# yangye1098/Speech-Denoising-Diffusion-Model-2

Hardware: AMD Instinct MI355X
Metric: denoised audio sec/sec, 1000-step UNetModified2 @16kHz (higher is better)
Workload: dtype bf16; 1 GPU; UNetModified2 config_unet.json, linear 1e-6..1e-3, T=1000, 16x16448-sample chunks per GPU, condition_in; model=UNetModified2, global_batch=16, seq_len=16448, parallelism=dp1, lane_rows=16

## Files before the change

### speech-denoising-diffusion-model-2_amd/csrc/conv_deep.hip

```cpp
#include "conv_common.h"
#include "conv_tile_cfg.h"
#include "kernels.h"

namespace sddm {

__device__ __attribute__((aligned(256))) unsigned char g_deep_zero[256];

constexpr int kDeepMaxChunks = 10;

#ifdef SDDM_STAMPS_ISSUE
#define DS_W(a) SDDM_STAMP(a, 1)
#define DS_STG(a) SDDM_STAMP(a, 2)
#define DS_ISSUED(a) SDDM_STAMP(a, 3)
#define DS_LANDED(a) SDDM_STAMP(a, 4)
#define DS_XFORM(a) SDDM_STAMP(a, 5)
#define DS_KLOOP(a) SDDM_STAMP(a, 6)
#define DS_STORED(a) do {} while (0)
#define DS_STATS(a) do {} while (0)
#else
#define DS_W(a) do {} while (0)
#define DS_STG(a) do {} while (0)
#define DS_ISSUED(a) SDDM_STAMP(a, 1)
#define DS_LANDED(a) SDDM_STAMP(a, 2)
#define DS_XFORM(a) SDDM_STAMP(a, 3)
// ... 62 lines not shown
    {128, 0, 8, 16, 32, 16, 96, 96, 96, 0, 0, 0, 1, 0, 8, 32, 0},
    {128, 0, 8, 16, 32, 16, 96, 0, 96, 96, 96, 2, 1, 0, 4, 32, 0},
    {64, 1, 4, 16, 64, 16, 96, 0, 96, 0, 0, 0, 0, 0, 4, 32, 1},
    {64, 0, 8, 8, 32, 8, 128, 0, 160, 0, 0, 0, 1, 0, 4, 32, 1},
    {64, 0, 8, 8, 32, 8, 160, 0, 160, 128, 0, 2, 1, 0, 4, 32, 1},
    {32, 1, 8, 4, 16, 4, 160, 0, 160, 0, 0, 0, 0, 0, 4, 32, 1},
    {32, 0, 8, 4, 16, 4, 160, 0, 160, 0, 0, 0, 1, 0, 4, 32, 1},
    {32, 0, 8, 4, 16, 4, 160, 0, 160, 0, 0, 1, 1, 0, 4, 32, 1},
    {32, 0, 8, 4, 16, 4, 160, 160, 160, 0, 0, 0, 1, 0, 4, 32, 1},
    {32, 0, 8, 4, 16, 4, 160, 0, 160, 160, 160, 2, 1, 0, 4, 32, 1},
    {64, 0, 8, 8, 32, 8, 160, 0, 160, 0, 0, 0, 0, 1, 4, 32, 1},
};
static constexpr int kNDeepShapes = (int)(sizeof(kDeepShapes) / sizeof(kDeepShapes[0]));

template <typename T, bool S2, int MT, int NW, int D, int NB, int SH>
__global__ __launch_bounds__(64 * NW, 8 / NW) void conv_deep_kernel(ConvArgs a) {
  extern __shared__ __attribute__((aligned(16))) char smem[];
  constexpr ConvShape SC = kDeepShapes[SH];
  constexpr bool CS = SH > 0;
  SDDM_SHAPE_GEO(SC, CS, S2, a)
  constexpr int NT = 64 * NW;
  constexpr int ES = (int)sizeof(T);
  constexpr int UPP = 2 * ES;
  constexpr int UPL = ES / 2;
  constexpr int VE = 16 / ES;
  constexpr int FP = MT / 16, FC = NB / 16, NBP = NB + 4;
  constexpr int TPP = NB / 4;
  constexpr int PPI = NT / TPP;
  constexpr int EIT = (MT + PPI - 1) / PPI;
  static_assert(NB == 16 || NB == 32 || NB == 64, "16, 32 or 64 output channels per block");
  constexpr int SLOTS = (NW == 8 && MT >= 128) ? 4 : NW;

  int tile, b, zb;
  if (a.deep_zin) xcd_block<true>(gNT, gCout / NB, tile, b, zb);
  else xcd_block<false>(gNT, gCout / NB, tile, b, zb);
  const int tid = threadIdx.x, lane = tid & 63, g = lane >> 4;
  const int wv = __builtin_amdgcn_readfirstlane(tid >> 6);
  const int n0 = zb * NB;
  const int ty = tile / gTX, tx = tile - ty * gTX;
  const int y0 = ty * gTR, x0 = tx * gTW;
  const int npv = gTR * gTW;
  const DeepGeo geo = deep_geo(S2, gTR, gTW, MT);
  const int HC = geo.HC, PLB = geo.PLB, PLR = geo.PLR;
  const int Cin = gCA + gCB, nck = Cin / 32, npl = Cin / VE, plA = gCA / VE;
  const int RC = gRes == 2 ? gRCA + gRCB : 0, rck = RC / 32, nplr = RC / VE, plRA = gRCA / VE;
  const bool gn = gGN, ident = gRes == 1;
  const DeepLds lay = deep_layout<T, MT, NW, NB>(geo, Cin, RC);
  float* gsc = (float*)(smem + lay.gsc);
  const int res_off = npl * PLB;
  const int img_in = gHi * gWi, img_out = gHo * gWo;
  const char* srcA = (const char*)a.srcA + (size_t)b * img_in * gCA * ES;
  const char* srcB = (const char*)(gCB ? a.srcB : a.srcA) + (size_t)b * img_in * gCB * ES;
  const char* zero = (const char*)g_deep_zero;
  const int* tdp = a.t_dev ? a.t_dev : (const int*)g_deep_zero;
  const int t_step = *tdp;
  const int t_now = a.temb_per_b ? b : t_step;
  SDDM_STAMP(a, 0);

  const int ec4 = (tid & (TPP - 1)) * 4;
  GNLoadT<DeepGN<NW>::GK> gl;
  const GNFuse gf{a.gstA, a.gtilesA, a.gntileA, a.gstB, a.gtilesB, a.gntileB, a.gamma, a.beta, a.groups, a.eps};
  gl.issue(gf, b, gCA, gCB, gn, a.bias);
  const int ns3 = nck * 9, ns = ns3 + rck;
  const int nj = wv < ns ? (ns - wv + NW - 1) / NW : 0;
  const int s_last = wv + NW * max(nj - 1, 0);
  const int cb0 = n0 / 16;
  const T* wbase = (const T*)a.wgt_f + (size_t)lane * 8;
  const T* rbase = (const T*)a.res_wgt_f + (size_t)lane * 8;
  auto wfrag = [&](int s, int fc) -> Frag<T> {
    const T* p = s < ns3 ? wbase + ((size_t)(cb0 + fc) * ns3 + s) * 512
                         : rbase + ((size_t)(cb0 + fc) * rck + (s - ns3)) * 512;
    return load_frag<T>((const char*)p);
  };
  Frag<T> wa[D][FC];
#pragma unroll
  for (int d = 0; d < D; ++d)
#pragma unroll
    for (int fc = 0; fc < FC; ++fc) wa[d][fc] = SDDM_DEEP_DBG(32) ? Frag<T>{} : wfrag(min(wv + NW * d, s_last), fc);
  DS_W(a);
  f32x4 idr[EIT];
  {
    const T* rsrc = (const T*)a.res_src + (size_t)b * img_out * gCout + n0 + ec4;
#pragma unroll
    for (int it = 0; it < EIT; ++it) {
      const int p = min(it * PPI + tid / TPP, npv - 1), py = p / gTW, px = p - py * gTW;
      const T* rp = ident ? rsrc + ((y0 + py) * gWo + (x0 + px)) * gCout : (const T*)g_deep_zero;
      idr[it] = load4<T>(rp);
    }
  }
  auto dma = [&](const char* src, char* dst) {
    __builtin_amdgcn_global_load_lds((const __attribute__((address_space(1))) void*)src,
                                     (__attribute__((address_space(3))) void*)dst, 16, 0, 0);
  };
  unsigned inb = 0;
  {
    const float rHC = 1.0f / (float)HC;
    for (int r = 0; r < geo.NCH; ++r) {
      const int hp = r * 64 + lane, hy = fdivi(hp, rHC), hx = hp - hy * HC;
      int iy, ix;
      bool ok;
      if (S2) {
        iy = 2 * y0 - 1 + hy; ix = 2 * x0 - 1 + hx;
        ok = iy >= 0 && iy < gHi && ix >= 0 && ix < gWi;
      } else {
        iy = y0 - 1 + hy; ix = x0 - 1 + hx;
        ok = iy >= 0 && iy < gHo && ix >= 0 && ix < gWo;
        if (gUp) { iy >>= 1; ix >>= 1; }
      }
      ok = ok && hp < geo.HP;
      inb |= ok ? 1u << r : 0u;
      const unsigned pix = ok ? (unsigned)(iy * gWi + ix) : 0u;
      const char* pa = ok ? srcA + pix * (unsigned)(gCA * ES) : zero;
      const char* pb = ok ? srcB + pix * (unsigned)(gCB * ES) - plA * 16 : zero;
      const unsigned step = ok ? 16u : 0u;
      char* dl = smem + r * 1024;
      for (int q = wv; q < npl; q += NW)
        if (!SDDM_DEEP_DBG(4)) dma((q < plA ? pa : pb) + q * step, dl + q * PLB);
    }
  }
  if (rck) {
    const char* rawA = (const char*)a.rawA + (size_t)b * img_out * gRCA * ES;
    const char* rawB = (const char*)(gRCB ? a.rawB : a.rawA) + (size_t)b * img_out * gRCB * ES;
    for (int r = 0; r < geo.NCR; ++r) {
      const int p = r * 64 + lane, py = p / gTW, px = p - py * gTW;
      const int pix = p < npv ? (y0 + py) * gWo + (x0 + px) : -1;
      const unsigned oa = (unsigned)pix * (unsigned)(gRCA * ES), ob = (unsigned)pix * (unsigned)(gRCB * ES);
      for (int q = wv; q < nplr; q += NW) {
        const char* src = q < plRA ? rawA + oa + q * 16 : rawB + ob + (q - plRA) * 16;
        dma(pix >= 0 ? src : zero, smem + res_off + q * PLR + r * 1024);
      }
    }
  }
  DS_STG(a);
  float bb[4], sshift;
  {
    const float* trow = a.temb ? a.temb + (size_t)t_now * a.temb_ld : a.bias;
#pragma unroll
    for (int i = 0; i < 4; ++i) {
      const float bv = a.bias[n0 + ec4 + i], tv = trow[n0 + ec4 + i];
      bb[i] = bv + (a.temb ? tv : 0.f);
    }
    const int cs = n0 + (tid & (NB - 1));
    const float sbv = a.bias[cs], stv = trow[cs];
    sshift = sbv + (a.temb ? stv : 0.f);
  }
  DS_ISSUED(a);

  if (gn) gl.finish(gf, b, gCA, gCB, gsc, gsc + Cin);
  dma_sync();
  DS_LANDED(a);

  if (gn) {
    for (int q0 = wv; q0 < npl; q0 += 2 * NW) {
      const bool two = q0 + NW < npl;
      const int q1 = two ? q0 + NW : q0;
      float s0[VE], h0[VE], s1[VE], h1[VE];
#pragma unroll
      for (int j = 0; j < VE; j += 4) {
        const f32x4 x0 = *(const f32x4*)(gsc + q0 * VE + j), y0 = *(const f32x4*)(gsc + Cin + q0 * VE + j);
        const f32x4 x1 = *(const f32x4*)(gsc + q1 * VE + j), y1 = *(const f32x4*)(gsc + Cin + q1 * VE + j);
#pragma unroll
// ... 58 lines not shown
  }
  DS_KLOOP(a);

  lds_sync();
  float* red = (float*)smem;
  auto put = [&](int slot) {
#pragma unroll
    for (int fp = 0; fp < FP; ++fp) {
      const int p = fp * 16 + (lane & 15);
#pragma unroll
      for (int fc = 0; fc < FC; ++fc) *(f32x4*)(red + (slot * MT + p) * NBP + fc * 16 + 4 * g) = acc[fp][fc];
    }
  };
  if (SLOTS < NW) {
    if (wv >= SLOTS) put(wv - SLOTS);
    lds_sync();
    if (wv < SLOTS) {
#pragma unroll
      for (int fp = 0; fp < FP; ++fp) {
        const int p = fp * 16 + (lane & 15);
#pragma unroll
        for (int fc = 0; fc < FC; ++fc) acc[fp][fc] += *(const f32x4*)(red + (wv * MT + p) * NBP + fc * 16 + 4 * g);
      }
      put(wv);
    }
  } else {
    put(wv);
  }
  lds_sync();

  float sn = 0.f, s1[4], s2[4];
#pragma unroll
  for (int i = 0; i < 4; ++i) { s1[i] = 0.f; s2[i] = 0.f; }
  T* out = (T*)a.out + (size_t)b * img_out * gCout + n0 + ec4;
#pragma unroll
  for (int it = 0; it < EIT; ++it) {
    const int p = it * PPI + tid / TPP;
    if (p < npv) {
      const int py = p / gTW, px = p - py * gTW;
      f32x4 s = *(const f32x4*)(red + p * NBP + ec4);
#pragma unroll
      for (int w = 1; w < SLOTS; ++w) s += *(const f32x4*)(red + (w * MT + p) * NBP + ec4);
      float d[4];
#pragma unroll
      for (int i = 0; i < 4; ++i) d[i] = s[i] + idr[it][i];
      store4<T>(out + ((y0 + py) * gWo + (x0 + px)) * gCout, d[0] + bb[0], d[1] + bb[1], d[2] + bb[2], d[3] + bb[3]);
#pragma unroll
      for (int i = 0; i < 4; ++i) {
        s1[i] += d[i];
        s2[i] += d[i] * d[i];
      }
      sn += 1.f;
    }
  }
  DS_STORED(a);
  if (a.stats) {
    auto wred = [](float x) {
      if constexpr (TPP == 4) x += dpp_f32<0x124>(x);
      if constexpr (TPP <= 8) x += dpp_f32<0x128>(x);
      x += __shfl_xor(x, 16);
      return x + __shfl_xor(x, 32);
    };
    const float tn = wred(sn);
    float t1[4], t2[4];
#pragma unroll
    for (int i = 0; i < 4; ++i) { t1[i] = wred(s1[i]); t2[i] = wred(s2[i]); }
    lds_sync();
    float* xs = red;
    if (lane < TPP)
#pragma unroll
      for (int i = 0; i < 4; ++i) {
        float* e = xs + (wv * NB + ec4 + i) * 3;
        e[0] = tn; e[1] = t1[i]; e[2] = t2[i];
      }
    lds_sync();
    if (tid < NB) {
      float n = 0.f, u1 = 0.f, u2 = 0.f;
#pragma unroll
      for (int r = 0; r < NW; ++r) {
        const float* e = xs + (r * NB + tid) * 3;
        n += e[0]; u1 += e[1]; u2 += e[2];
      }
      float* dst = a.stats + (((size_t)b * gNT + tile) * gCout + n0 + tid) * 2;
      dst[0] = (sshift + u1 / n) * n;
      dst[1] = fmaxf(u2 - u1 * u1 / n, 0.f);
    }
  }
  DS_STATS(a);
  SDDM_STAMP(a, 7);
}

template <typename T, int MT, int NW>
static int deep_ring(int steps_per_wave) {
  if (sizeof(T) == 4 || NW == 4) return 8 / (int)(sizeof(T) == 4 ? 2 : 1);
  if (steps_per_wave <= 8 || MT >= 128) return 8;
  return 12;
}

template <typename T, bool S2, int MT, int NW, int NB, int SH = 0>
static hipError_t deep_go(const ConvArgs& a, int B, hipStream_t s, size_t* lo) {
  const int Cin = a.CA + a.CB, RC = a.res_mode == 2 ? a.RCA + a.RCB : 0;
  const int nck = Cin / 32, rck = RC / 32;
  const DeepGeo geo = deep_geo(S2, a.TR, a.TW, MT);
  const DeepLds lay = deep_layout<T, MT, NW, NB>(geo, Cin, RC);
  const bool fits = geo.NCH <= kDeepMaxChunks && geo.NCR <= 2;
  if (lo) {
    *lo = fits ? (size_t)lay.total : (size_t)1 << 40;
    return hipSuccess;
  }
  if (!fits || a.TR * a.TW > MT || a.Cout % NB || Cin % 32 || Cin > 1000 || RC % 32 || a.CA % 32)
    return hipErrorInvalidValue;
  if (lay.total > kLdsBytes) return hipErrorInvalidValue;
  const dim3 grid = xcd_grid(a.n_tiles, B, a.Cout / NB), blk(64 * NW);
  const int D = deep_ring<T, MT, NW>((nck * 9 + rck + NW - 1) / NW);
#define SDDM_RING(DV)                                                                         \
  if (D == DV) {                                                                              \
    hipLaunchKernelGGL((conv_deep_kernel<T, S2, MT, NW, DV, NB, SH>), grid, blk, lay.total, s, a); \
    return hipGetLastError();                                                                 \
  }
  if constexpr (NB == 64) {
    if constexpr (sizeof(T) == 4) {
      return hipErrorInvalidValue;
    } else {
      hipLaunchKernelGGL((conv_deep_kernel<T, S2, MT, NW, 4, NB, SH>), grid, blk, lay.total, s, a);
      return hipGetLastError();
    }
  } else if constexpr (SH > 0) {
    constexpr ConvShape c = kDeepShapes[SH];
    constexpr int spw = (((c.CA + c.CB) / 32) * 9 + (c.res == 2 ? (c.RCA + c.RCB) / 32 : 0) + NW - 1) / NW;
    constexpr int DS = (NW == 4 || MT >= 128 || spw <= 8) ? 8 : 12;
    SDDM_RING(DS)
  } else if constexpr (sizeof(T) == 4) {
    SDDM_RING(4)
  } else if constexpr (NW == 4 || MT >= 128) {
    SDDM_RING(8)
  } else {
    SDDM_RING(8) SDDM_RING(12)
  }
#undef SDDM_RING
  return hipErrorInvalidValue;
// ... 64 lines not shown
```

### speech-denoising-diffusion-model-2_amd/csrc/kernels.h

```cpp
#pragma once
#include <hip/hip_runtime.h>
#include <stdint.h>

namespace sddm {

struct EmbedArgs {
  const float* noise_levels;
  const float* table;
  int time_step_mode;
  int R;
  int dim;
  const float* emb_vec;
  const float* w1; const float* b1;
  const float* w2; const float* b2;
  const float* pw; const float* pb;
  int SC;
  float* out;
};
hipError_t launch_embed(const EmbedArgs& a, hipStream_t s);

struct GNSrc { const float* stats; int C; int tiles; int n_tile; };
struct GNArgs {
  GNSrc a, b;
  const float* gamma; const float* beta;
// ... 16 lines not shown
};
hipError_t launch_conv_in(int dtype, const ConvInArgs& a, int B, hipStream_t s);

struct GNFuse;
struct ConvArgs {
  const void* srcA; const void* srcB; int CA, CB;
  int Hi, Wi;
  int Ho, Wo;
  int upsample;
  int TR, TW, tiles_x, n_tiles;
  const float* gstA; int gtilesA, gntileA;
  const float* gstB; int gtilesB, gntileB;
  const float* gamma; const float* beta; int groups; float eps;
  const void* wgt;
  const float* bias;
  const float* temb; int temb_ld; const int* t_dev; int temb_per_b;
  int Cout;
  int res_mode;
  const void* res_src;
  const void* rawA; const void* rawB; int RCA, RCB;
  const void* res_wgt;
  void* out;
  float* stats;
  int deep_zin;
  int deep_nw;
  int deep_nb;
  unsigned long long* stamps;
  int dbg;
  const void* wgt_t;
  const void* res_wgt_t;
  const void* wgt_f;
  const void* res_wgt_f;
};

struct ChainArgs {
  const void* x;
  void* out;
  const void* wgt[5];
  const void* res_wgt;
  const float* bias[5];
  const float* gamma[4]; const float* beta[4];
  const float* temb[2];
  int temb_ld; const int* t_dev; int temb_per_b;
  int C, H, W, groups; float eps;
};
hipError_t launch_conv_chain(int dtype, const ChainArgs& a, int B, hipStream_t s);

struct TileCfg { int wpx, wco, fp, fc; };
int conv_tile_ncfg();
TileCfg conv_tile_cfg(int cfg);
hipError_t launch_conv_tile(int dtype, int cfg, bool s2, const ConvArgs& a, int B, hipStream_t s);
size_t conv_tile_lds_bytes(int cfg, bool s2, const ConvArgs& a);

hipError_t launch_conv_deep(int dtype, int mt, bool s2, const ConvArgs& a, int B, hipStream_t s);
size_t conv_deep_lds_bytes(int dtype, int mt, bool s2, const ConvArgs& a);
int conv_deep_ring_depth(int dtype, int mt, int nw, int ksteps, int nb);

constexpr int kLdsBytes = 160 * 1024;

hipError_t launch_conv_strip(int dtype, int nblk, int mpi, int SR, const ConvArgs& a, int B, hipStream_t s);
size_t conv_strip_lds_bytes(int dtype, int nblk, int mpi, const ConvArgs& a);

struct TransCoef {
  const float* betas; const float* alphas; const float* sqrt_alpha_bar; const float* pnc;
  const float* sigma; const float* sgamma; const float* ssh; const float* sqrt_delta;
  const float* c_xt; const float* c_yt; const float* c_epst; const float* sde;
// ... 79 lines not shown
```

### speech-denoising-diffusion-model-2_amd/csrc/sddm_runtime.cpp

```cpp
#include <hip/hip_runtime.h>

#include <algorithm>
#include <cstdarg>
#include <cstdlib>
#include <cstdio>
#include <cstring>
#include <functional>
#include <map>
#include <set>
#include <memory>
#include <string>
#include <vector>

#include "../../include/sddm_hip.h"
#include "json_mini.h"
#include "kernels.h"
#include "q_kernels.h"
#include "stft_kernels.h"
#include "sddm_common.h"

namespace sddm {
int compute_schedule(const std::string& schedule, int T, double linear_start, double linear_end,
                     float* out);
}
// ... 134 lines not shown
      s[n + ".block2.block.0.bias"] = {L.cout};
      s[n + ".block2.block.3.weight"] = {L.cout, L.cout, 3, 3};
      s[n + ".block2.block.3.bias"] = {L.cout};
      if (L.cin != L.cout) {
        s[n + ".res_conv.weight"] = {L.cout, L.cin, 1, 1};
        s[n + ".res_conv.bias"] = {L.cout};
      }
    } else if (L.kind == 2 || L.kind == 3) {
      s[n + ".conv.weight"] = {L.cout, L.cin, 3, 3};
      s[n + ".conv.bias"] = {L.cout};
    } else if (L.kind == 0) {
      s[n + ".weight"] = {L.cout, L.cin, 3, 3};
      s[n + ".bias"] = {L.cout};
    } else {
      s[n + ".block.0.weight"] = {L.cin};
      s[n + ".block.0.bias"] = {L.cin};
      s[n + ".block.3.weight"] = {L.cout, L.cin, 3, 3};
      s[n + ".block.3.bias"] = {L.cout};
    }
  }
  return s;
}

struct Param { std::vector<int64_t> shape; std::vector<float> data; bool loaded = false; };
struct Tensor { void* p = nullptr; int C = 0, H = 0, W = 0; float* stats = nullptr; int tiles = 0, n_tile = 0; };
struct Op {
  int cls;
  double bytes, flops;
  std::function<hipError_t(hipStream_t)> run;
  std::string name = "";
  std::function<hipError_t(hipStream_t, int)> run_dbg = nullptr;
  std::string kname = "";
  std::string kinst = "";
};
struct ProfAcc { double ms = 0; int64_t n = 0; double bytes = 0, flops = 0; };

struct RunState {
  const float* cond = nullptr;
  float* x = nullptr;
  const float* temb = nullptr;
  int temb_per_b = 0;
  int* t_dev = nullptr;
  int final_mode = 0;
  float* eps_out = nullptr;
  uint64_t seed = 0;
  int64_t row_offset = 0;
  const float* noise = nullptr;
  int64_t noise_ld = 0;
};

static constexpr int kStreams = 4;
static constexpr int kMaxLanes = 64;

struct Lane {
  int B = 0, row0 = 0, idx = 0;
  Arena arena;
  std::vector<Op> ops;
  RunState rs;
  size_t off_temb_fwd = 0, off_cond = 0, off_x = 0;
  hipGraphExec_t gexec = nullptr;
  hipGraph_t graph = nullptr;
  int g_K = 0, g_gen = -1;
  ~Lane() {
    if (gexec) (void)hipGraphExecDestroy(gexec);
    if (graph) (void)hipGraphDestroy(graph);
    arena.reset();
// ... 257 lines not shown
    const int TW = std::min(a.Wo, mt);
    if (mt % TW || a.Wo % TW) continue;
    const int TR = std::min(mt / TW, a.Ho);
    if (a.Ho % TR) continue;
    if (TR * TW < mt && mt > 32) continue;
    a.TR = TR; a.TW = TW; a.tiles_x = a.Wo / TW; a.n_tiles = a.tiles_x * (a.Ho / TR);
    for (int nw : {8, 4}) {
      a.deep_nw = nw;
      if (conv_deep_lds_bytes(dt, mt, s2, a) > kLdsBytes) continue;
      const int blocks = a.n_tiles * B * nz, per_round = 256 * (nw == 4 ? 2 : 1);
      cs.push_back({mt, nw, TR, TW, a.tiles_x, a.n_tiles, blocks, (blocks + per_round - 1) / per_round});
    }
  }
  if (cs.empty()) return false;
  const Cand* pick = nullptr;
  const int fm = want_mt ? want_mt : force_mt, fn = want_mt ? want_nw : force_nw;
  for (const Cand& c : cs)
    if (c.mt == fm && c.nw == fn) pick = &c;
  if (!pick) {
    pick = &cs[0];
    for (const Cand& c : cs) {
      if (c.rounds != pick->rounds) { if (c.rounds < pick->rounds) pick = &c; continue; }
      if (c.nw != pick->nw) { if (c.nw > pick->nw) pick = &c; continue; }
      if (c.mt < pick->mt) pick = &c;
    }
  }
  ch.strip = 0; ch.mt = pick->mt; ch.nw = pick->nw; ch.nb = nb; ch.ckb = (a.CA + a.CB) / 32;
  ch.TR = pick->TR; ch.TW = pick->TW; ch.tiles_x = pick->tiles_x; ch.n_tiles = pick->n_tiles;
  return true;
}

static int deep_zin(const ConvArgs& a, int B, size_t es) {
  static const int force = std::getenv("SDDM_DEEP_ZIN") ? std::atoi(std::getenv("SDDM_DEEP_ZIN")) : -1;
  if (force >= 0) return force;
  const double in = (double)B * a.Hi * a.Wi * (a.CA + a.CB) * es;
  const double w = (double)a.Cout * ((a.CA + a.CB) * 9 + (a.res_mode == 2 ? a.RCA + a.RCB : 0)) * es;
  return in >= w ? 1 : 0;
}

static bool choose_tile(int dt, int B, ConvArgs a, bool s2, ConvChoice& ch, int want = -1) {
  if (dt == DT_F32) return false;
  static const int force = std::getenv("SDDM_TILE_CFG") ? std::atoi(std::getenv("SDDM_TILE_CFG")) : -1;
  static const bool off = std::getenv("SDDM_NO_TILE") != nullptr;
  if (off) return false;
  const int fw = want >= 0 ? want : force;
  struct Cand { int cfg, TR, TW, tiles_x, n_tiles, blocks, area; };
  std::vector<Cand> cs;
  for (int cfg = 0; cfg < conv_tile_ncfg(); ++cfg) {
    const TileCfg t = conv_tile_cfg(cfg);
    const int MT = t.wpx * t.fp * 16, NB = t.wco * t.fc * 16;
    if (a.Cout % NB) continue;
    const int TW = std::min(a.Wo, MT);
    if (MT % TW || a.Wo % TW) continue;
    const int TR = std::min(MT / TW, a.Ho);
    if (a.Ho % TR) continue;
    if (TR * TW < MT && (TR != a.Ho || TW != a.Wo)) continue;
    a.TR = TR; a.TW = TW; a.tiles_x = a.Wo / TW; a.n_tiles = a.tiles_x * (a.Ho / TR);
    if (conv_tile_lds_bytes(cfg, s2, a) > kLdsBytes) continue;
    cs.push_back({cfg, TR, TW, a.tiles_x, a.n_tiles, a.n_tiles * B * (a.Cout / NB), TR * TW * NB});
  }
  if (cs.empty()) return false;
  const Cand* pick = nullptr;
  for (const Cand& c : cs)
    if (c.cfg == fw) pick = &c;
  if (!pick) {
    for (const Cand& c : cs) {
      if (!pick) { pick = &c; continue; }
// ... 16 lines not shown
  a.Hi = up ? Ho / 2 : (s2 ? Ho * 2 : Ho); a.Wi = up ? Wo / 2 : (s2 ? Wo * 2 : Wo);
  static const int env_mpi = std::getenv("SDDM_STRIP_MPI") ? std::atoi(std::getenv("SDDM_STRIP_MPI")) : 0;
  static const int env_blocks = std::getenv("SDDM_STRIP_BLOCKS") ? std::atoi(std::getenv("SDDM_STRIP_BLOCKS")) : 0;
  if (kind == 2) {
    ConvChoice t = ch;
    if (choose_tile(dt, B, a, s2, t, ka) && t.tile == ka) { ch = t; return true; }
  }
  if (!s2 && (Wo == 128 || Wo == 64) && std::getenv("SDDM_NO_STRIP") == nullptr && (kind == 0 || kind == 1)) {
    const int nbs[2] = {(Cout % 64 == 0) ? 64 : 32, 32};
    for (int mpi : {256, 128}) {
      if (env_mpi && mpi != env_mpi) continue;
      const int TRs = mpi / Wo;
      if (Ho % TRs) continue;
      for (int ni = 0; ni < 2; ++ni) {
        const int nb = nbs[ni];
        if (conv_strip_lds_bytes(dt, nb, mpi, a) > kLdsBytes) continue;
        const int nz = (Cout + nb - 1) / nb;
        int SR = 0;
        const int target = env_blocks ? env_blocks : 256;
        for (int m = 32; m >= 2; m /= 2) {
          const int sr = TRs * m;
          if (Ho % sr) continue;
          SR = sr;
          if ((Ho / sr) * B * nz >= target) break;
        }
        if (SR == 0) continue;
        ch.strip = 1; ch.nblk = nb; ch.SR = SR; ch.mpi = mpi;
        ch.TR = SR; ch.TW = Wo; ch.tiles_x = 1; ch.n_tiles = Ho / SR;
        return true;
      }
    }
  }
  if (want_mt == 0 && kind != 3 && choose_tile(dt, B, a, s2, ch)) return true;
  return choose_deep(dt, B, a, s2, ch, want_mt, want_nw, want_nb);
}

static int build_lane(sddm_ctx* c, Lane& L) {
  const int B = L.B;
  Lane* lp = &L;
  const int dt = c->dtype;
  const size_t es = dtype_size(dt);
  const UNetCfg& u = c->ucfg;
  const int N = c->num_samples, W = u.seg, S = u.stride;
  const int F = (N - W) / S + 1;
  L.ops.clear();
  L.arena.reset();
  Arena& A = L.arena;

  struct TRes { size_t p, st; int C, H, W, tiles, n_tile; };
  std::vector<TRes> tres;
  auto new_tensor = [&](int C, int H, int Wd, int tiles, int n_tile) -> int {
    TRes t;
    t.p = A.reserve((size_t)B * H * Wd * C * es);
    t.st = A.reserve(sizeof(float) * (size_t)B * tiles * C * 2);
    t.C = C; t.H = H; t.W = Wd; t.tiles = tiles; t.n_tile = n_tile;
    tres.push_back(t);
    return (int)tres.size() - 1;
  };
  struct GNRes { int a, b; std::string w; };
  std::vector<GNRes> gres;
  auto new_gn = [&](int xa, int xb, const std::string& w) -> int {
    gres.push_back({xa, xb, w});
    return (int)gres.size() - 1;
  };
  L.off_temb_fwd = A.reserve(sizeof(float) * (size_t)B * std::max(c->SC, 1));
  L.off_cond = A.reserve(sizeof(float) * (size_t)B * N);
  L.off_x = A.reserve(sizeof(float) * (size_t)B * N);

  enum { ST_CONVIN, ST_GN, ST_CONV, ST_FINAL };
  struct Step {
    int type = 0;
    std::string w;
    std::string rb;
    int srcA = -1, srcB = -1, gn = -1, out = -1;
    int s2 = 0, up = 0, res_mode = 0, rawA = -1, rawB = -1, cout = 0;
    bool temb = false;
    ConvChoice ch;
  };
  std::vector<Step> prog;
  const int PB = std::max(1, c->lane_rows);
  const sddm_ctx::TuneTable* tuned = nullptr;
  for (const auto& tt : c->tunes)
    if (tt.B == PB && tt.N == N && tt.dtype == dt) { tuned = &tt; break; }
  if (!tuned && dt == DT_F16)
    for (const auto& tt : c->tunes)
      if (tt.B == PB && tt.N == N && tt.dtype == DT_BF16) { tuned = &tt; break; }
  auto pick = [&](const std::string& name, int Cin, int RC, int res_mode, int Ho, int Wo, int cout, bool s2, bool up,
                  ConvChoice& ch) {
    int wm = 0, wn = 0, wb = 0, kind = 0, ka = 0;
    if (tuned) {
      auto it = tuned->deep_tune.find(name);
      if (it != tuned->deep_tune.end()) { wm = it->second.first; wn = it->second.second; kind = 3; }
      auto kt = tuned->kern_tune.find(name);
      if (kt != tuned->kern_tune.end()) {
        kind = kt->second.kind; ka = kt->second.a;
        if (kind == 3) { wm = kt->second.a; wn = kt->second.b; wb = kt->second.c; }
      }
    }
    const bool chain = kind == 4 && dt != DT_F32;
    if (kind == 4) kind = 0;
    const bool ok = choose_conv(dt, PB, Cin, RC, res_mode, Ho, Wo, cout, s2, up, ch, wm, wn, kind, ka, wb);
    ch.chain = chain ? 1 : 0;
    return ok;
  };
  const int TRin = 512 / W;
  if (u.inner != 32 || 512 % W || F % TRin || (TRin + 1) * S + W + 2 > 1024)
    FAIL(SDDM_ERR_NOT_IMPLEMENTED, "conv_in needs inner_channel 32 and segment_len dividing 512 (got %d, %d)", u.inner, W);
  const int t0 = new_tensor(u.inner, F, W, F / TRin, TRin * W);
  { Step st; st.type = ST_CONVIN; st.out = t0; prog.push_back(st); }

  auto res_block = [&](const std::string& n, int xa, int xb, int cin, int cout) -> int {
    const int H = tres[xa].H, Wd = tres[xa].W;
    ConvChoice c1, c2;
    if (!pick(n + ".block1", cin, 0, 0, H, Wd, cout, false, false, c1)) return -1;
    if (!pick(n + ".block2", cout, cin, cin != cout ? 2 : 1, H, Wd, cout, false, false, c2)) return -1;
    const int g1 = new_gn(xa, xb, n + ".block1");
    const int h = new_tensor(cout, H, Wd, c1.n_tiles, c1.TR * c1.TW);
    { Step st; st.type = ST_CONV; st.w = n + ".block1"; st.rb = n; st.srcA = xa; st.srcB = xb; st.gn = g1;
      st.out = h; st.cout = cout; st.temb = true; st.ch = c1; prog.push_back(st); }
    const int g2 = new_gn(h, -1, n + ".block2");
    const int o = new_tensor(cout, H, Wd, c2.n_tiles, c2.TR * c2.TW);
    { Step st; st.type = ST_CONV; st.w = n + ".block2"; st.rb = n; st.srcA = h; st.gn = g2; st.out = o;
      st.cout = cout; st.res_mode = cin != cout ? 2 : 1; st.rawA = xa; st.rawB = xb; st.ch = c2; prog.push_back(st); }
    return o;
  };
  std::vector<LayerDesc> downs, mid, ups;
  unet_layers(u, &downs, &mid, &ups);
  std::vector<int> feats{t0};
  int cur = t0;
  for (size_t i = 1; i < downs.size(); ++i) {
    const LayerDesc& L = downs[i];
    if (L.kind == 1) {
// ... 7 lines not shown
      Step st; st.type = ST_CONV; st.w = L.name; st.srcA = cur; st.out = o; st.s2 = 1; st.cout = L.cout; st.ch = ch;
      prog.push_back(st);
      cur = o;
    }
    if (cur < 0) FAIL(SDDM_ERR_SHAPE, "no tile for %s", L.name.c_str());
    feats.push_back(cur);
  }
  for (const LayerDesc& L : mid) {
    cur = res_block(L.name, cur, -1, L.cin, L.cout);
    if (cur < 0) FAIL(SDDM_ERR_SHAPE, "no tile for %s", L.name.c_str());
  }
  for (const LayerDesc& L : ups) {
    if (L.kind == 1) {
      const int skip = feats.back();
      feats.pop_back();
      if (tres[skip].H != tres[cur].H || tres[skip].W != tres[cur].W)
        FAIL(SDDM_ERR_SHAPE, "skip/upsample size mismatch at %s (torch.cat would raise)", L.name.c_str());
      cur = res_block(L.name, cur, skip, L.cin, L.cout);
      if (cur < 0) FAIL(SDDM_ERR_SHAPE, "no tile for %s", L.name.c_str());
    } else {
      const int H = tres[cur].H * 2, Wd = tres[cur].W * 2;
      ConvChoice ch;
      if (!pick(L.name, tres[cur].C, 0, 0, H, Wd, L.cout, false, true, ch)) FAIL(SDDM_ERR_SHAPE, "no tile for %s", L.name.c_str());
      const int o = new_tensor(L.cout, H, Wd, ch.n_tiles, ch.TR * ch.TW);
      Step st; st.type = ST_CONV; st.w = L.name; st.srcA = cur; st.out = o; st.up = 1; st.cout = L.cout; st.ch = ch;
      prog.push_back(st);
      cur = o;
    }
  }
  const int gf = new_gn(cur, -1, "final_conv");
  { Step st; st.type = ST_FINAL; st.srcA = cur; st.gn = gf; prog.push_back(st); }

  SDDM_HIP_CHECK(A.commit());

  auto TT = [&](int i) {
    Tensor t;
    if (i < 0) return t;
    const TRes& r = tres[i];
    t.p = A.base + r.p; t.stats = A.at<float>(r.st); t.C = r.C; t.H = r.H; t.W = r.W;
    t.tiles = r.tiles; t.n_tile = r.n_tile;
    return t;
  };
  auto WF = [&](const std::string& k) { return c->warena.at<float>(c->woff.at(k)); };
  auto WV = [&](const std::string& k) { return (const void*)(c->warena.base + c->woff.at(k)); };
  auto conv_args = [&](const Step& st, ConvArgs& a, double& bytes, double& flops) -> int {
    a = ConvArgs{};
    const Tensor sa = TT(st.srcA), sb = TT(st.srcB), o = TT(st.out);
    a.srcA = sa.p; a.srcB = sb.p; a.CA = sa.C; a.CB = sb.C;
    a.Hi = sa.H; a.Wi = sa.W; a.Ho = o.H; a.Wo = o.W; a.upsample = st.up;
    a.Cout = st.cout; a.out = o.p; a.stats = o.stats;
    if (st.gn >= 0) {
      const GNRes& gr = gres[st.gn];
      const Tensor ga = TT(gr.a), gb = TT(gr.b);
      a.gstA = ga.stats; a.gtilesA = ga.tiles; a.gntileA = ga.n_tile;
      a.gstB = gb.stats; a.gtilesB = gb.tiles; a.gntileB = gb.n_tile;
      a.gamma = WF(gr.w + ".gamma"); a.beta = WF(gr.w + ".beta"); a.groups = u.groups; a.eps = 1e-5f;
      const int Ct = ga.C + gb.C;
      if (Ct % u.groups || (gb.C && ga.C % (Ct / u.groups)) || 256 % u.groups)
        FAIL(SDDM_ERR_SHAPE, "GroupNorm(%d, %d) at %s: unsupported grouping", u.groups, Ct, gr.w.c_str());
    }
    a.wgt = WV(st.w + ".w"); a.bias = WF(st.w + ".b");
    a.wgt_t = c->woff.count(st.w + ".w_t") ? WV(st.w + ".w_t") : nullptr;
    a.wgt_f = WV(st.w + ".w_f");
    a.res_mode = st.res_mode;
    const int Cin = a.CA + a.CB;
    bytes = (double)B * a.Hi * a.Wi * Cin * es + (double)B * a.Ho * a.Wo * a.Cout * es +
// ... 74 lines not shown
      const Tensor o = TT(st.out);
      a.out = o.p; a.stats = o.stats; a.TR = TRin;
      const double bytes = (double)B * N * 4 * 2 + (double)B * F * W * u.inner * es;
      const double flops = 2.0 * B * F * W * u.inner * 18;
#ifdef SDDM_STAMPS
      if (const char* sn = std::getenv("SDDM_STAMPS"))
        if (std::string(sn) == "downs.0") {
          if (!c->stamp_buf) SDDM_HIP_CHECK(hipMalloc(&c->stamp_buf, sizeof(unsigned long long) * 8 * 65536));
          a.stamps = c->stamp_buf;
          c->stamp_blocks = (int64_t)(F / TRin) * B;
        }
#endif
      L.ops.push_back({0, bytes, flops, [lp, a, dt, B](hipStream_t s) {
                          ConvInArgs x = a;
                          x.cond = lp->rs.cond; x.x = lp->rs.x; x.t_dev = lp->rs.t_dev;
                          return launch_conv_in(dt, x, B, s);
                        }, "downs.0"});
      L.ops.back().kname = std::string("conv_in_kernel<") + dt_name(dt) + ">";
      L.ops.back().kinst = L.ops.back().kname;
    } else if (st.type == ST_CONV) {
      ConvArgs a;
      double bytes = 0, flops = 0;
      if (const int r = conv_args(st, a, bytes, flops)) return r;
      const int Cin = a.CA + a.CB;
      const ConvChoice ch = st.ch;
      const bool s2 = st.s2 != 0;
      const bool temb = st.temb;
      if (std::getenv("SDDM_PRINT_SHAPES"))
        fprintf(stderr, "SHAPE %s %s%d s2=%d TR=%d TW=%d Ho=%d Wo=%d CA=%d CB=%d Cout=%d RCA=%d RCB=%d res=%d gn=%d up=%d mt=%d nw=%d nb=%d nblk=%d mpi=%d SR=%d ntiles=%d\n",
                st.w.c_str(), ch.strip ? "strip" : (ch.tile >= 0 ? "tile" : "deep"), ch.tile >= 0 ? ch.tile : ch.mt, s2 ? 1 : 0,
                a.TR, a.TW, a.Ho, a.Wo, a.CA, a.CB, a.Cout, a.RCA, a.RCB, a.res_mode, a.gamma ? 1 : 0, a.upsample ? 1 : 0,
                ch.mt, ch.nw, ch.nb, ch.nblk, ch.mpi, ch.SR, a.n_tiles);
      const int toff = temb ? c->temb_off.at(st.rb) : 0;
#ifdef SDDM_STAMPS
      if (const char* sn = std::getenv("SDDM_STAMPS")) {
        if (st.w == sn) {
          if (!c->stamp_buf) SDDM_HIP_CHECK(hipMalloc(&c->stamp_buf, sizeof(unsigned long long) * 8 * 65536));
          SDDM_HIP_CHECK(hipMemset(c->stamp_buf, 0, sizeof(unsigned long long) * 8 * 65536));
          a.stamps = c->stamp_buf;
          if (const char* f = std::getenv("SDDM_STAMPS_DBG")) a.dbg = std::atoi(f);
          int nb = 32;
          if (ch.tile >= 0) { const TileCfg tc = conv_tile_cfg(ch.tile); nb = tc.wco * tc.fc * 16; }
          c->stamp_blocks = ch.strip ? (int64_t)(a.Ho / ch.SR) * B * ((a.Cout + ch.nblk - 1) / ch.nblk)
                                     : (int64_t)a.n_tiles * B * (a.Cout / (ch.tile >= 0 ? nb : ch.nb));
        }
      }
#endif
      L.ops.push_back({2, bytes, flops, [ctx, lp, a, s2, ch, dt, B, temb, toff](hipStream_t s) {
                          ConvArgs x = a;
                          if (temb) {
                            x.temb = lp->rs.temb + toff;
                            x.temb_ld = ctx->SC;
                            x.temb_per_b = lp->rs.temb_per_b;
                            x.t_dev = lp->rs.t_dev;
                          }
                          if (ch.strip) return launch_conv_strip(dt, ch.nblk, ch.mpi, ch.SR, x, B, s);
                          if (ch.tile >= 0) return launch_conv_tile(dt, ch.tile, s2, x, B, s);
                          x.deep_zin = deep_zin(x, B, dtype_size(dt)); x.deep_nw = ch.nw; x.deep_nb = ch.nb;
                          return launch_conv_deep(dt, ch.mt, s2, x, B, s);
                        }, st.w + (ch.strip ? "[strip]" : (ch.tile >= 0 ? "[tile" + std::to_string(ch.tile) + "]"
                                                                         : "[deep" + std::to_string(ch.mt) + "_" + std::to_string(ch.nw) + "_" + std::to_string(ch.nb) + "]"))});
      {
        char kn[160];
        if (ch.strip)
          snprintf(kn, sizeof(kn), "conv_strip_kernel<%s,%d,%d,%d,%d>", dt_name(dt), ch.nblk / 16, a.Wo, Cin, ch.mpi);
        else if (ch.tile >= 0) {
          const TileCfg tc = conv_tile_cfg(ch.tile);
          snprintf(kn, sizeof(kn), "conv_tile_kernel<%s,%d,%d,%d,%d,%d> (tile%d)", dt_name(dt), s2 ? 1 : 0, tc.wpx, tc.wco,
                   tc.fp, tc.fc, ch.tile);
        } else
          snprintf(kn, sizeof(kn), "conv_deep_kernel<%s,%d,%d,%d,%d>", dt_name(dt), s2 ? 1 : 0, ch.mt, ch.nw, ch.nb);
        L.ops.back().kname = kn;
        char ki[192];
        if (ch.strip)
          snprintf(ki, sizeof(ki), "conv_strip_kernel<%s,%d,%d,%d,%d,%d,%d>", dt_name(dt), ch.nblk / 16, a.Wo, Cin,
                   ch.mpi, a.res_mode, a.gamma ? 1 : 0);
        else if (ch.tile >= 0)
          snprintf(ki, sizeof(ki), "%s", kn);
        else
          snprintf(ki, sizeof(ki), "conv_deep_kernel<%s,%d,%d,%d,%d,%d>", dt_name(dt), s2 ? 1 : 0, ch.mt, ch.nw,
                   conv_deep_ring_depth(dt, ch.mt, ch.nw, (Cin / 32) * 9 + (a.res_mode == 2 ? (a.RCA + a.RCB) / 32 : 0), ch.nb),
                   ch.nb);
        L.ops.back().kinst = ki;
      }
      {
        auto base = L.ops.back().run;
        ConvArgs a0 = a;
        L.ops.back().run_dbg = [lp, ctx, a0, s2, ch, dt, B, temb, toff](hipStream_t s, int fl) {
          ConvArgs x = a0;
          if (temb && !(fl & 4)) { x.temb = lp->rs.temb + toff; x.temb_ld = ctx->SC; x.temb_per_b = lp->rs.temb_per_b; x.t_dev = lp->rs.t_dev; }
          if (fl & 1) x.stats = nullptr;
          if (fl & 2) x.gamma = nullptr;
          if (fl & 4) x.res_mode = 0;
          x.dbg = fl;
          if (ch.strip) return launch_conv_strip(dt, ch.nblk, ch.mpi, ch.SR, x, B, s);
          if (ch.tile >= 0) return launch_conv_tile(dt, ch.tile, s2, x, B, s);
          x.deep_zin = deep_zin(x, B, dtype_size(dt)); x.deep_nw = ch.nw; x.deep_nb = ch.nb;
          return launch_conv_deep(dt, ch.mt, s2, x, B, s);
        };
        (void)base;
      }
    } else {
      FinalArgs f{};
      const Tensor src = TT(st.srcA);
      f.src = src.p; f.C = src.C;
      {
        const GNRes& gr = gres[st.gn];
        const Tensor ga = TT(gr.a);
        f.gst = ga.stats; f.gtiles = ga.tiles; f.gntile = ga.n_tile;
        f.gamma = WF("final_conv.gamma"); f.beta = WF("final_conv.beta"); f.groups = u.groups; f.eps = 1e-5f;
        if (ga.C % u.groups || 256 % u.groups) FAIL(SDDM_ERR_SHAPE, "final GroupNorm grouping");
      }
      f.w = WF("final_conv.w");
      f.bias = c->params.at("final_conv.block.3.bias").data[0];
      static const int env_ft = std::getenv("SDDM_FINAL_FT") ? std::atoi(std::getenv("SDDM_FINAL_FT")) : 0;
      f.N = N; f.F = F; f.W = W; f.S = S; f.FT = (env_ft == 16 && F % 16 == 0) ? 16 : (F % 8 == 0 ? 8 : 2);
      if (F % f.FT || W % S) FAIL(SDDM_ERR_SHAPE, "final tile: frames %d, segment %d/%d", F, W, S);
      f.co = c->coef();
      const double bytes = (double)B * F * W * src.C * es + (double)B * N * 4 * 3;
      const double flops = 2.0 * B * F * W * src.C * 9;
#ifdef SDDM_STAMPS
      if (const char* sn = std::getenv("SDDM_STAMPS"))
        if (std::string(sn) == "final_conv") {
          if (!c->stamp_buf) SDDM_HIP_CHECK(hipMalloc(&c->stamp_buf, sizeof(unsigned long long) * 8 * 65536));
          f.stamps = c->stamp_buf;
          c->stamp_blocks = (int64_t)(F / f.FT) * B;
        }
#endif
      L.ops.push_back({3, bytes, flops, [lp, f, dt, B](hipStream_t s) {
                          FinalArgs x = f;
// ... 733 lines not shown
  double ms = 0, bytes = 0, flops = 0;
  int64_t n = 0;
  for (size_t i = 0; i < c->op_acc.size() && i < ops.size(); ++i) {
    if (ops[i].cls != cls) continue;
    ms += c->op_acc[i].ms; bytes += c->op_acc[i].bytes; flops += c->op_acc[i].flops; n += c->op_acc[i].n;
  }
  if (avg_ms) *avg_ms = n ? ms / n : 0.0;
  if (launches) *launches = n;
  if (bytes_per_launch) *bytes_per_launch = n ? bytes / n : 0.0;
  if (flops_per_launch) *flops_per_launch = n ? flops / n : 0.0;
  return SDDM_OK;
}

int sddm_debug_stamps(sddm_ctx* c, void* host, int64_t max_blocks, int64_t* n_blocks) {
  if (!c || !host || !n_blocks) FAIL(SDDM_ERR_INVALID_ARG, "NULL argument");
  *n_blocks = 0;
  if (!c->stamp_buf) return SDDM_OK;
  const int64_t n = std::min<int64_t>(c->stamp_blocks, max_blocks);
  SDDM_HIP_CHECK(hipDeviceSynchronize());
  SDDM_HIP_CHECK(hipMemcpy(host, c->stamp_buf, sizeof(unsigned long long) * 8 * n, hipMemcpyDeviceToHost));
  *n_blocks = n;
  return SDDM_OK;
}

int sddm_profile_ops(sddm_ctx* c, char* buf, int64_t buflen) {
  if (!c || !buf || buflen < 3) FAIL(SDDM_ERR_INVALID_ARG, "NULL argument");
  const std::vector<Op>& ops = profiled_ops(c);
  std::string js = "[";
  char tmp[768];
  for (size_t i = 0; i < ops.size(); ++i) {
    const ProfAcc a = i < c->op_acc.size() ? c->op_acc[i] : ProfAcc{};
    snprintf(tmp, sizeof(tmp),
             "%s{\"name\": \"%s\", \"kernel\": \"%s\", \"inst\": \"%s\", \"cls\": %d, \"launches\": %lld, "
             "\"avg_ms\": %.6f, \"bytes\": %.0f, \"flops\": %.0f}",
             i ? ", " : "", ops[i].name.c_str(), ops[i].kname.c_str(), ops[i].kinst.c_str(), ops[i].cls, (long long)a.n,
             a.n ? a.ms / a.n : 0.0, ops[i].bytes, ops[i].flops);
    js += tmp;
  }
  js += "]";
  if ((int64_t)js.size() + 1 > buflen) FAIL(SDDM_ERR_INVALID_ARG, "buffer too small (%zu)", js.size() + 1);
  std::memcpy(buf, js.c_str(), js.size() + 1);
  return SDDM_OK;
}

}
```

Baseline: 25.63 audio_s/s.

## Store deep-conv-only intermediate tensors in channel-planar layout

Adds a planar activation layout (16-byte channel groups stored contiguously across pixels) for tensors that are produced and consumed only by deep conv kernels. The kernel's DMA gathers, residual loads and output stores switch strides per-operand via layout bits packed into deep_zin. The aim is more coalesced global loads and stores for the per-pixel 16-byte chunks that feed LDS. It also narrows chain-kernel selection to a single shape, adds a fallback when a forced deep config fails, and excludes fp32 NB=64 from the deep kernel, which changes kernel choice for other layers.

New measurement: 25.89 audio_s/s, median of 6. No clear change (+1.0%).

```diff
diff --git a/speech-denoising-diffusion-model-2_amd/csrc/conv_deep.hip b/speech-denoising-diffusion-model-2_amd/csrc/conv_deep.hip
--- a/speech-denoising-diffusion-model-2_amd/csrc/conv_deep.hip
+++ b/speech-denoising-diffusion-model-2_amd/csrc/conv_deep.hip
@@ -118,7 +118,7 @@
   constexpr int SLOTS = (NW == 8 && MT >= 128) ? 4 : NW;
 
   int tile, b, zb;
-  if (a.deep_zin) xcd_block<true>(gNT, gCout / NB, tile, b, zb);
+  if (a.deep_zin & kDeepZin) xcd_block<true>(gNT, gCout / NB, tile, b, zb);
   else xcd_block<false>(gNT, gCout / NB, tile, b, zb);
   const int tid = threadIdx.x, lane = tid & 63, g = lane >> 4;
   const int wv = __builtin_amdgcn_readfirstlane(tid >> 6);
@@ -138,6 +138,9 @@
   const char* srcA = (const char*)a.srcA + (size_t)b * img_in * gCA * ES;
   const char* srcB = (const char*)(gCB ? a.srcB : a.srcA) + (size_t)b * img_in * gCB * ES;
   const char* zero = (const char*)g_deep_zero;
+  const int lay_bits = a.deep_zin;
+  const unsigned pszA = lay_bits & kDeepPlA ? 16u : (unsigned)(gCA * ES), qszA = lay_bits & kDeepPlA ? (unsigned)img_in * 16u : 16u;
+  const unsigned pszB = lay_bits & kDeepPlB ? 16u : (unsigned)(gCB * ES), qszB = lay_bits & kDeepPlB ? (unsigned)img_in * 16u : 16u;
   const int* tdp = a.t_dev ? a.t_dev : (const int*)g_deep_zero;
   const int t_step = *tdp;
   const int t_now = a.temb_per_b ? b : t_step;
@@ -166,11 +169,14 @@
   DS_W(a);
   f32x4 idr[EIT];
   {
-    const T* rsrc = (const T*)a.res_src + (size_t)b * img_out * gCout + n0 + ec4;
+    const bool plr = (lay_bits & kDeepPlRes) != 0;
+    const int cr = n0 + ec4;
+    const T* rsrc = (const T*)a.res_src + (size_t)b * img_out * gCout + (plr ? (cr / VE) * (img_out * VE) + cr % VE : cr);
+    const int rpx = plr ? VE : gCout;
 #pragma unroll
     for (int it = 0; it < EIT; ++it) {
       const int p = min(it * PPI + tid / TPP, npv - 1), py = p / gTW, px = p - py * gTW;
-      const T* rp = ident ? rsrc + ((y0 + py) * gWo + (x0 + px)) * gCout : (const T*)g_deep_zero;
+      const T* rp = ident ? rsrc + ((y0 + py) * gWo + (x0 + px)) * rpx : (const T*)g_deep_zero;
       idr[it] = load4<T>(rp);
     }
   }
@@ -196,12 +202,12 @@
       ok = ok && hp < geo.HP;
       inb |= ok ? 1u << r : 0u;
       const unsigned pix = ok ? (unsigned)(iy * gWi + ix) : 0u;
-      const char* pa = ok ? srcA + pix * (unsigned)(gCA * ES) : zero;
-      const char* pb = ok ? srcB + pix * (unsigned)(gCB * ES) - plA * 16 : zero;
-      const unsigned step = ok ? 16u : 0u;
+      const unsigned stepA = ok ? qszA : 0u, stepB = ok ? qszB : 0u;
+      const char* pa = ok ? srcA + pix * pszA : zero;
+      const char* pb = ok ? srcB + pix * pszB - (size_t)plA * qszB : zero;
       char* dl = smem + r * 1024;
       for (int q = wv; q < npl; q += NW)
-        if (!SDDM_DEEP_DBG(4)) dma((q < plA ? pa : pb) + q * step, dl + q * PLB);
+        if (!SDDM_DEEP_DBG(4)) dma(q < plA ? pa + q * stepA : pb + q * stepB, dl + q * PLB);
     }
   }
   if (rck) {
@@ -210,9 +216,12 @@
     for (int r = 0; r < geo.NCR; ++r) {
       const int p = r * 64 + lane, py = p / gTW, px = p - py * gTW;
       const int pix = p < npv ? (y0 + py) * gWo + (x0 + px) : -1;
-      const unsigned oa = (unsigned)pix * (unsigned)(gRCA * ES), ob = (unsigned)pix * (unsigned)(gRCB * ES);
+      const unsigned oa = (unsigned)pix * (lay_bits & kDeepPlRawA ? 16u : (unsigned)(gRCA * ES));
+      const unsigned ob = (unsigned)pix * (lay_bits & kDeepPlRawB ? 16u : (unsigned)(gRCB * ES));
+      const unsigned qa = lay_bits & kDeepPlRawA ? (unsigned)img_out * 16u : 16u;
+      const unsigned qb = lay_bits & kDeepPlRawB ? (unsigned)img_out * 16u : 16u;
       for (int q = wv; q < nplr; q += NW) {
-        const char* src = q < plRA ? rawA + oa + q * 16 : rawB + ob + (q - plRA) * 16;
+        const char* src = q < plRA ? rawA + oa + q * qa : rawB + ob + (q - plRA) * qb;
         dma(pix >= 0 ? src : zero, smem + res_off + q * PLR + r * 1024);
       }
     }
@@ -337,7 +346,10 @@
   float sn = 0.f, s1[4], s2[4];
 #pragma unroll
   for (int i = 0; i < 4; ++i) { s1[i] = 0.f; s2[i] = 0.f; }
-  T* out = (T*)a.out + (size_t)b * img_out * gCout + n0 + ec4;
+  const bool plo = (lay_bits & kDeepPlOut) != 0;
+  const int co = n0 + ec4;
+  T* out = (T*)a.out + (size_t)b * img_out * gCout + (plo ? (co / VE) * (img_out * VE) + co % VE : co);
+  const int opx = plo ? VE : gCout;
 #pragma unroll
   for (int it = 0; it < EIT; ++it) {
     const int p = it * PPI + tid / TPP;
@@ -349,7 +361,7 @@
       float d[4];
 #pragma unroll
       for (int i = 0; i < 4; ++i) d[i] = s[i] + idr[it][i];
-      store4<T>(out + ((y0 + py) * gWo + (x0 + px)) * gCout, d[0] + bb[0], d[1] + bb[1], d[2] + bb[2], d[3] + bb[3]);
+      store4<T>(out + ((y0 + py) * gWo + (x0 + px)) * opx, d[0] + bb[0], d[1] + bb[1], d[2] + bb[2], d[3] + bb[3]);
 #pragma unroll
       for (int i = 0; i < 4; ++i) {
         s1[i] += d[i];
@@ -410,7 +422,7 @@
   const DeepLds lay = deep_layout<T, MT, NW, NB>(geo, Cin, RC);
   const bool fits = geo.NCH <= kDeepMaxChunks && geo.NCR <= 2;
   if (lo) {
-    *lo = fits ? (size_t)lay.total : (size_t)1 << 40;
+    *lo = fits && !(NB == 64 && sizeof(T) == 4) ? (size_t)lay.total : (size_t)1 << 40;
     return hipSuccess;
   }
   if (!fits || a.TR * a.TW > MT || a.Cout % NB || Cin % 32 || Cin > 1000 || RC % 32 || a.CA % 32)
diff --git a/speech-denoising-diffusion-model-2_amd/csrc/kernels.h b/speech-denoising-diffusion-model-2_amd/csrc/kernels.h
--- a/speech-denoising-diffusion-model-2_amd/csrc/kernels.h
+++ b/speech-denoising-diffusion-model-2_amd/csrc/kernels.h
@@ -72,6 +72,8 @@
   const void* wgt_f;
   const void* res_wgt_f;
 };
+
+enum : int { kDeepZin = 1, kDeepPlA = 2, kDeepPlB = 4, kDeepPlRawA = 8, kDeepPlRawB = 16, kDeepPlRes = 32, kDeepPlOut = 64 };
 
 struct ChainArgs {
   const void* x;
diff --git a/speech-denoising-diffusion-model-2_amd/csrc/sddm_runtime.cpp b/speech-denoising-diffusion-model-2_amd/csrc/sddm_runtime.cpp
--- a/speech-denoising-diffusion-model-2_amd/csrc/sddm_runtime.cpp
+++ b/speech-denoising-diffusion-model-2_amd/csrc/sddm_runtime.cpp
@@ -190,6 +190,7 @@
   std::function<hipError_t(hipStream_t, int)> run_dbg = nullptr;
   std::string kname = "";
   std::string kinst = "";
+  std::string layout = "";
 };
 struct ProfAcc { double ms = 0; int64_t n = 0; double bytes = 0, flops = 0; };
 
@@ -513,7 +514,7 @@
 
 static int deep_zin(const ConvArgs& a, int B, size_t es) {
   static const int force = std::getenv("SDDM_DEEP_ZIN") ? std::atoi(std::getenv("SDDM_DEEP_ZIN")) : -1;
-  if (force >= 0) return force;
+  if (force >= 0) return force ? 1 : 0;
   const double in = (double)B * a.Hi * a.Wi * (a.CA + a.CB) * es;
   const double w = (double)a.Cout * ((a.CA + a.CB) * 9 + (a.res_mode == 2 ? a.RCA + a.RCB : 0)) * es;
   return in >= w ? 1 : 0;
@@ -596,7 +597,8 @@
     }
   }
   if (want_mt == 0 && kind != 3 && choose_tile(dt, B, a, s2, ch)) return true;
-  return choose_deep(dt, B, a, s2, ch, want_mt, want_nw, want_nb);
+  if (choose_deep(dt, B, a, s2, ch, want_mt, want_nw, want_nb)) return true;
+  return want_mt != 0 && choose_conv(dt, B, Cin, RC, res_mode, Ho, Wo, Cout, s2, up, ch);
 }
 
 static int build_lane(sddm_ctx* c, Lane& L) {
@@ -661,7 +663,7 @@
         if (kind == 3) { wm = kt->second.a; wn = kt->second.b; wb = kt->second.c; }
       }
     }
-    const bool chain = kind == 4 && dt != DT_F32;
+    const bool chain = kind == 4 && dt != DT_F32 && cout == 160 && Ho == 8 && Wo == 4;
     if (kind == 4) kind = 0;
     const bool ok = choose_conv(dt, PB, Cin, RC, res_mode, Ho, Wo, cout, s2, up, ch, wm, wn, kind, ka, wb);
     ch.chain = chain ? 1 : 0;
@@ -735,6 +737,22 @@
   { Step st; st.type = ST_FINAL; st.srcA = cur; st.gn = gf; prog.push_back(st); }
 
   SDDM_HIP_CHECK(A.commit());
+
+  auto is_deep = [](const Step& s) { return s.type == ST_CONV && !s.ch.strip && s.ch.tile < 0 && !s.ch.chain; };
+  std::vector<char> planar(tres.size(), 0);
+  {
+    const char* e = std::getenv("SDDM_DEEP_PLANAR");
+    if (!e || std::atoi(e) != 0) {
+      std::vector<char> other(tres.size(), 0);
+      for (const Step& s : prog) {
+        if (is_deep(s)) { planar[s.out] = 1; continue; }
+        for (int t : {s.srcA, s.srcB, s.rawA, s.rawB})
+          if (t >= 0) other[t] = 1;
+      }
+      for (size_t i = 0; i < tres.size(); ++i) planar[i] = planar[i] && !other[i];
+    }
+  }
+  auto PL = [&](int i) { return i >= 0 && planar[i]; };
 
   auto TT = [&](int i) {
     Tensor t;
@@ -875,6 +893,16 @@
                 a.TR, a.TW, a.Ho, a.Wo, a.CA, a.CB, a.Cout, a.RCA, a.RCB, a.res_mode, a.gamma ? 1 : 0, a.upsample ? 1 : 0,
                 ch.mt, ch.nw, ch.nb, ch.nblk, ch.mpi, ch.SR, a.n_tiles);
       const int toff = temb ? c->temb_off.at(st.rb) : 0;
+      int lay = 0;
+      std::string lay_js;
+      if (is_deep(st)) {
+        const struct { int t, bit; const char* nm; } lt[] = {
+            {st.srcA, kDeepPlA, "A"}, {st.srcB, kDeepPlB, "B"},
+            {st.res_mode == 2 ? st.rawA : -1, kDeepPlRawA, "rawA"}, {st.res_mode == 2 ? st.rawB : -1, kDeepPlRawB, "rawB"},
+            {st.res_mode == 1 ? st.rawA : -1, kDeepPlRes, "res"}, {st.out, kDeepPlOut, "out"}};
+        for (const auto& e : lt)
+          if (PL(e.t)) { lay |= e.bit; lay_js += std::string(lay_js.empty() ? "\"" : ", \"") + e.nm + "\""; }
+      }
 #ifdef SDDM_STAMPS
       if (const char* sn = std::getenv("SDDM_STAMPS")) {
         if (st.w == sn) {
@@ -889,7 +917,7 @@
         }
       }
 #endif
-      L.ops.push_back({2, bytes, flops, [ctx, lp, a, s2, ch, dt, B, temb, toff](hipStream_t s) {
+      L.ops.push_back({2, bytes, flops, [ctx, lp, a, s2, ch, dt, B, temb, toff, lay](hipStream_t s) {
                           ConvArgs x = a;
                           if (temb) {
                             x.temb = lp->rs.temb + toff;
@@ -899,7 +927,7 @@
                           }
                           if (ch.strip) return launch_conv_strip(dt, ch.nblk, ch.mpi, ch.SR, x, B, s);
                           if (ch.tile >= 0) return launch_conv_tile(dt, ch.tile, s2, x, B, s);
-                          x.deep_zin = deep_zin(x, B, dtype_size(dt)); x.deep_nw = ch.nw; x.deep_nb = ch.nb;
+                          x.deep_zin = deep_zin(x, B, dtype_size(dt)) | lay; x.deep_nw = ch.nw; x.deep_nb = ch.nb;
                           return launch_conv_deep(dt, ch.mt, s2, x, B, s);
                         }, st.w + (ch.strip ? "[strip]" : (ch.tile >= 0 ? "[tile" + std::to_string(ch.tile) + "]"
                                                                          : "[deep" + std::to_string(ch.mt) + "_" + std::to_string(ch.nw) + "_" + std::to_string(ch.nb) + "]"))});
@@ -914,6 +942,7 @@
         } else
           snprintf(kn, sizeof(kn), "conv_deep_kernel<%s,%d,%d,%d,%d>", dt_name(dt), s2 ? 1 : 0, ch.mt, ch.nw, ch.nb);
         L.ops.back().kname = kn;
+        L.ops.back().layout = lay_js;
         char ki[192];
         if (ch.strip)
           snprintf(ki, sizeof(ki), "conv_strip_kernel<%s,%d,%d,%d,%d,%d,%d>", dt_name(dt), ch.nblk / 16, a.Wo, Cin,
@@ -929,7 +958,7 @@
       {
         auto base = L.ops.back().run;
         ConvArgs a0 = a;
-        L.ops.back().run_dbg = [lp, ctx, a0, s2, ch, dt, B, temb, toff](hipStream_t s, int fl) {
+        L.ops.back().run_dbg = [lp, ctx, a0, s2, ch, dt, B, temb, toff, lay](hipStream_t s, int fl) {
           ConvArgs x = a0;
           if (temb && !(fl & 4)) { x.temb = lp->rs.temb + toff; x.temb_ld = ctx->SC; x.temb_per_b = lp->rs.temb_per_b; x.t_dev = lp->rs.t_dev; }
           if (fl & 1) x.stats = nullptr;
@@ -938,7 +967,7 @@
           x.dbg = fl;
           if (ch.strip) return launch_conv_strip(dt, ch.nblk, ch.mpi, ch.SR, x, B, s);
           if (ch.tile >= 0) return launch_conv_tile(dt, ch.tile, s2, x, B, s);
-          x.deep_zin = deep_zin(x, B, dtype_size(dt)); x.deep_nw = ch.nw; x.deep_nb = ch.nb;
+          x.deep_zin = deep_zin(x, B, dtype_size(dt)) | lay; x.deep_nw = ch.nw; x.deep_nb = ch.nb;
           return launch_conv_deep(dt, ch.mt, s2, x, B, s);
         };
         (void)base;
@@ -1738,9 +1767,9 @@
     const ProfAcc a = i < c->op_acc.size() ? c->op_acc[i] : ProfAcc{};
     snprintf(tmp, sizeof(tmp),
              "%s{\"name\": \"%s\", \"kernel\": \"%s\", \"inst\": \"%s\", \"cls\": %d, \"launches\": %lld, "
-             "\"avg_ms\": %.6f, \"bytes\": %.0f, \"flops\": %.0f}",
+             "\"avg_ms\": %.6f, \"bytes\": %.0f, \"flops\": %.0f, \"layout\": [%s]}",
              i ? ", " : "", ops[i].name.c_str(), ops[i].kname.c_str(), ops[i].kinst.c_str(), ops[i].cls, (long long)a.n,
-             a.n ? a.ms / a.n : 0.0, ops[i].bytes, ops[i].flops);
+             a.n ? a.ms / a.n : 0.0, ops[i].bytes, ops[i].flops, ops[i].layout.c_str());
     js += tmp;
   }
   js += "]";
```
